# snuspl/parallax

Hardware: NVIDIA H100
Metric: lm1b_words_per_sec (higher is better)
Workload: dtype bf16

## Files before the change

parallax_b200/ops/fused.py:

```python
import ctypes

import torch

from . import lib as _lib, check as _check, register_signatures

_vp, _i, _f = ctypes.c_void_p, ctypes.c_int, ctypes.c_float
register_signatures({
    "px_lstm_cell_fwd": (_i, [_vp, _vp, _vp, _vp, _vp, _i, _i, _f, _i, _vp]),
    "px_lstm_cell_bwd": (_i, [_vp, _vp, _vp, _vp, _vp, _vp, _i, _i, _i, _vp]),
    "px_lstm_dm_cell_bwd": (_i, [_vp] * 7 + [_i, _i, _i, _i, _vp]),
    "px_sampled_softmax": (_i, [_vp, _vp, _vp, _vp, _vp, _vp, _vp, _vp, _i, _i, _i, _vp]),
    "px_sampled_softmax_dot": (_i, [_vp, _vp, _vp, _i, _vp, _vp, _vp, _vp, _vp, _vp, _i, _i, _i,
                                    _vp]),
    "px_ssm_bwd": (_i, [_vp, _vp, _vp, _vp, _i, _vp, _vp, _f, _vp, _vp, _vp, _i, _vp, _i, _i, _i,
                        _vp]),
})
_DT = {torch.float32: 0, torch.bfloat16: 1}


def _p(t):
    return _vp(t.data_ptr())


def _stream():
    return _vp(torch.cuda.current_stream().cuda_stream)


def _count(n=1):
    from ..parallel import nvops
    nvops.launches["n"] += n


def _acc(t):
    return t if t.dtype == torch.float64 else t.float()


BWD_BN = 16


def _fused_bwd_ok(dt, Bsz, S, P, W_P):
    return (dt == torch.bfloat16 and Bsz % 128 == 0 and S % BWD_BN == 0 and P % 64 == 0 and
            W_P.is_contiguous() and W_P.data_ptr() % 16 == 0)


def lstm_layer_reference(x, Wx, Wh, bias, W_P, c0, h0, forget_bias=1.0):
    T, Bsz, E = x.shape
    S = W_P.shape[0]
    xw = torch.addmm(bias, x.reshape(T * Bsz, E), Wx).view(T, Bsz, 4 * S)
    c, h, outs = _acc(c0), h0, []
    for t in range(T):
        gates = _acc(torch.addmm(xw[t], h, Wh))
        i, j, f, o = gates.split(S, dim=1)
        c = torch.sigmoid(f + forget_bias) * c + torch.sigmoid(i) * torch.tanh(j)
        m = (torch.sigmoid(o) * torch.tanh(c)).to(x.dtype)
        h = m @ W_P
        outs.append(h)
    return torch.stack(outs), c, h


class _LSTMLayerFn(torch.autograd.Function):

    @staticmethod
    def forward(ctx, x, W, Wh, bias, W_P, c0, h0, forget_bias):
        L = _lib()
        T, Bsz, E = x.shape
        S, P = W_P.shape
        dt = x.dtype
        dev = x.device
        x = x.contiguous()
        stacked = Wh is None
        ctx.stacked = stacked
        ctx.param_refs = (W, bias, W_P)
        if stacked:
            Wx, Wh = W.detach()[:E], W.detach()[E:]
        else:
            Wx = W
        if any(ctx.needs_input_grad) and not _fused_bwd_ok(dt, Bsz, S, P, W_P):
            from . import sinks
            cur = torch.cuda.current_stream(dev)
            ws = sinks.side_stream(dev)
            ws.wait_stream(cur)
            with torch.cuda.stream(ws):
                ctx.WPT = W_P.detach().t().contiguous()
                ctx.WPT_ev = torch.cuda.Event()
                ctx.WPT_ev.record(ws)
            ctx.WPT.record_stream(cur)
        xw = torch.addmm(bias, x.view(T * Bsz, E), Wx).view(T, Bsz, 4 * S)
        act = torch.empty(T, Bsz, 4 * S, dtype=dt, device=dev)
        c_all = torch.empty(T + 1, Bsz, S, dtype=torch.float32, device=dev)
        m_all = torch.empty(T, Bsz, S, dtype=dt, device=dev)
        h_all = torch.empty(T + 1, Bsz, P, dtype=dt, device=dev)
        c_all[0].copy_(c0)
        h_all[0].copy_(h0)
        st = _stream()
        for t in range(T):
            gpre = xw[t].addmm_(h_all[t], Wh)
            _check(L.px_lstm_cell_fwd(_p(gpre), _p(c_all[t]), _p(act[t]),
                                      _p(c_all[t + 1]), _p(m_all[t]), Bsz, S,
                                      float(forget_bias), _DT[dt], st), "lstm_cell_fwd")
            torch.mm(m_all[t], W_P, out=h_all[t + 1])
        _count(T)
        ctx.save_for_backward(x, Wx, Wh, W_P, act, c_all, m_all, h_all)
        ctx.dims = (T, Bsz, E, S, P)
        return h_all[1:], c_all[T].clone(), h_all[T].clone()

    @staticmethod
    def backward(ctx, dH, dcT, dhT):
        from . import sinks
        L = _lib()
        x, Wx, Wh, W_P, act, c_all, m_all, h_all = ctx.saved_tensors
        T, Bsz, E, S, P = ctx.dims
        stacked = ctx.stacked
        W_ref, bias_ref, WP_ref = ctx.param_refs
        dt, dev = x.dtype, x.device
        dH = dH.contiguous()
        dgates = torch.empty(T, Bsz, 4 * S, dtype=dt, device=dev)
        dh_tot = torch.empty(T, Bsz, P, dtype=dt, device=dev)
        dc = torch.zeros(Bsz, S, dtype=torch.float32, device=dev) if dcT is None \
            else dcT.float().clone()
        dh_rec = None if dhT is None else dhT.to(dt)
        fused = _fused_bwd_ok(dt, Bsz, S, P, W_P)
        dm = None if fused else torch.empty(Bsz, S, dtype=dt, device=dev)
        cur = torch.cuda.current_stream(dev)
        if not fused:
            cur.wait_event(ctx.WPT_ev)
            WPT = ctx.WPT
        from . import gemm as _gemm
        use_tc = (dt == torch.bfloat16 and Bsz % 128 == 0 and P % 64 == 0 and
                  (4 * S) % 1024 == 0 and Wh.is_contiguous())
        WhT = None if use_tc else Wh.t().contiguous()
        st = _stream()

        def sink_of(ref, shape):
            s_ = sinks.get(ref)
            if s_ is not None and s_.dtype == dt and tuple(s_.shape) == tuple(shape):
                return s_, True
            return torch.empty(shape, dtype=dt, device=dev), False
        if stacked:
            dW, w_sunk = sink_of(W_ref, (E + P, 4 * S))
            dWx_o, dWh_o = dW[:E], dW[E:]
        else:
            dWx_o, w_sunk = sink_of(W_ref, (E, 4 * S))
            dWh_o = torch.empty(P, 4 * S, dtype=dt, device=dev)
        dbias_o, b_sunk = sink_of(bias_ref, (4 * S,))
        dWP_o, p_sunk = sink_of(WP_ref, (S, P))
        ws = sinks.side_stream(dev)
        ws2 = sinks.side_stream(dev, 1)
        if dh_rec is None:
            dh_tot[T - 1].copy_(dH[T - 1])
        else:
            torch.add(dH[T - 1], dh_rec, out=dh_tot[T - 1])
        for t in range(T - 1, -1, -1):
            if fused:
                _check(L.px_lstm_dm_cell_bwd(_p(dh_tot[t]), _p(W_P), _p(dc), _p(act[t]),
                                             _p(c_all[t]), _p(c_all[t + 1]), _p(dgates[t]), Bsz,
                                             S, P, BWD_BN, st), "lstm_dm_cell_bwd")
            else:
                torch.mm(dh_tot[t], WPT, out=dm)
                _check(L.px_lstm_cell_bwd(_p(dm), _p(dc), _p(act[t]), _p(c_all[t]),
                                          _p(c_all[t + 1]), _p(dgates[t]), Bsz, S, _DT[dt], st),
                       "lstm_cell_bwd")
            if t > 0:
                if use_tc:
                    _gemm.gemm_tn(dgates[t], Wh, addend=dH[t - 1], splits=8, bn=64,
                                  out=dh_tot[t - 1])
                else:
                    torch.addmm(dH[t - 1], dgates[t], WhT, out=dh_tot[t - 1])
            else:
                dh_rec = _gemm.gemm_tn(dgates[0], Wh, splits=8, bn=64) if use_tc \
                    else torch.mm(dgates[0], WhT)
        _count(T)
        dg2 = dgates.view(T * Bsz, 4 * S)
        ws2.wait_stream(cur)
        with torch.cuda.stream(ws2):
            torch.sum(dg2, 0, out=dbias_o)
        ev_b = torch.cuda.Event()
        ev_b.record(ws2)
        dgates.record_stream(ws2)
        dbias_o.record_stream(ws2)
        dx = (dg2 @ Wx.t()).view(T, Bsz, E)
        ws.wait_stream(cur)
        with torch.cuda.stream(ws):
            torch.mm(h_all[:T].reshape(-1, P).t(), dg2, out=dWh_o)
            torch.mm(x.reshape(-1, E).t(), dg2, out=dWx_o)
            torch.mm(m_all.reshape(-1, S).t(), dh_tot.view(-1, P), out=dWP_o)
        ev = torch.cuda.Event()
        ev.record(ws)
        for t_ in (dgates, dh_tot, x, h_all, m_all, dWh_o, dWx_o, dbias_o, dWP_o):
            t_.record_stream(ws)
        outs, plain = [], False
        for ref, o, sunk, e_ in ((W_ref, dW if stacked else dWx_o, w_sunk, ev),
                                 (bias_ref, dbias_o, b_sunk, ev_b), (WP_ref, dWP_o, p_sunk, ev)):
            if sunk:
                sinks.deliver(ref, e_)
                outs.append(None)
            else:
                outs.append(o)
                plain = True
        if plain or not stacked:
            cur.wait_event(ev)
            cur.wait_event(ev_b)
        dW_out, dbias, dW_P = outs
        return dx, dW_out, None if stacked else dWh_o, dbias, dW_P, dc, dh_rec, None


def lstm_layer(x, Wx, Wh, bias, W_P, c0, h0, forget_bias=1.0):
    if x.is_cuda and x.dtype in _DT:
        return _LSTMLayerFn.apply(x, Wx, Wh, bias, W_P, c0, h0, forget_bias)
    return lstm_layer_reference(x, Wx, Wh, bias, W_P, c0, h0, forget_bias)


def lstm_layer_stacked(x, W, bias, W_P, c0, h0, forget_bias=1.0):
    E = x.shape[-1]
    if x.is_cuda and x.dtype in _DT:
        return _LSTMLayerFn.apply(x, W, None, bias, W_P, c0, h0, forget_bias)
    return lstm_layer_reference(x, W[:E], W[E:], bias, W_P, c0, h0, forget_bias)


def sampled_softmax_reference(inputs, true_w, samp_w, true_b, samp_b, logq_true,
                              logq_samp, targets, sampled):
    true_logits = _acc((inputs * true_w).sum(-1)) + _acc(true_b) - logq_true
    samp_logits = _acc(inputs @ samp_w.t()) + (_acc(samp_b) - logq_samp)
    hits = targets.unsqueeze(1) == sampled.unsqueeze(0)
    samp_logits = samp_logits.masked_fill(hits, float("-inf"))
    lse = torch.logsumexp(torch.cat([true_logits.unsqueeze(1), samp_logits], 1), 1)
    return lse - true_logits


class _SampledSoftmaxFn(torch.autograd.Function):
    @staticmethod
    def forward(ctx, inputs, true_w, samp_w, true_b, samp_b, logq_true, logq_samp,
                targets, sampled):
        L = _lib()
        N, S = inputs.shape[0], samp_w.shape[0]
        dt = inputs.dtype
        logits = inputs @ samp_w.t()
        true_dot = (inputs.float() * true_w.float()).sum(-1)
        adj_t = (true_b.float() - logq_true).contiguous()
        adj_s = (samp_b.float() - logq_samp).contiguous()
        loss = torch.empty(N, dtype=torch.float32, device=inputs.device)
        dtrue = torch.empty(N, dtype=torch.float32, device=inputs.device)
        tg = targets.to(torch.int64).contiguous()
        sm = sampled.to(torch.int64).contiguous()
        _check(L.px_sampled_softmax(_p(logits), _p(true_dot), _p(adj_t), _p(adj_s), _p(tg),
                                    _p(sm), _p(loss), _p(dtrue), N, S, _DT[dt], _stream()),
               "sampled_softmax")
        _count(1)
        ctx.save_for_backward(inputs, true_w, samp_w, logits, dtrue)
        return loss

    @staticmethod
    def backward(ctx, g):
        inputs, true_w, samp_w, probs, dtrue = ctx.saved_tensors
        dt = inputs.dtype
        g = g.float()
        gt = (g * dtrue).unsqueeze(1)
        d_inputs = ((probs @ samp_w).float() * g.unsqueeze(1) +
                    gt * true_w.float()).to(dt)
        gi = (inputs.float() * g.unsqueeze(1)).to(dt)
        d_samp_w = probs.t() @ gi
        d_true_w = (gt * inputs.float()).to(dt)
        d_samp_b = (probs.float().t() @ g) if probs.dtype == torch.float32 else \
            torch.mm(probs.t(), g.to(dt).unsqueeze(1), out_dtype=torch.float32).squeeze(1)
        d_true_b = gt.squeeze(1)
        return d_inputs, d_true_w, d_samp_w, d_true_b, d_samp_b, None, None, None, None


def sampled_softmax_loss(inputs, true_w, samp_w, true_b, samp_b, logq_true, logq_samp,
                         targets, sampled):
    if inputs.is_cuda and inputs.dtype in _DT and samp_w.shape[0] <= 256 * 64:
        return _SampledSoftmaxFn.apply(inputs, true_w.to(inputs.dtype),
                                       samp_w.to(inputs.dtype), true_b, samp_b,
                                       logq_true, logq_samp, targets, sampled)
    return sampled_softmax_reference(inputs, true_w, samp_w, true_b, samp_b, logq_true,
                                     logq_samp, targets, sampled)


def _head_forward(inputs, w_all, adj, targets, sampled):
    N, S = inputs.shape[0], w_all.shape[0] - inputs.shape[0]
    P = inputs.shape[1]
    logits = inputs @ w_all[N:].t()
    if inputs.is_cuda:
        loss = torch.empty(N, dtype=torch.float32, device=inputs.device)
        dtrue = torch.empty(N, dtype=torch.float32, device=inputs.device)
        _check(_lib().px_sampled_softmax_dot(
            _p(logits), _p(inputs), _p(w_all), P, _p(adj), _vp(adj.data_ptr() + 4 * N),
            _p(targets), _p(sampled), _p(loss), _p(dtrue), N, S, _DT[inputs.dtype], _stream()),
            "sampled_softmax_dot")
        _count(1)
        return logits, loss, dtrue
    tl = (inputs.float() * w_all[:N].float()).sum(-1) + adj[:N]
    a = logits.float() + adj[N:]
    a = a.masked_fill(targets.unsqueeze(1) == sampled.unsqueeze(0), float("-inf"))
    mx = torch.maximum(a.max(1).values, tl)
    e, et = torch.exp(a - mx.unsqueeze(1)), torch.exp(tl - mx)
    denom = e.sum(1) + et
    return (e / denom.unsqueeze(1)).to(inputs.dtype), mx + torch.log(denom) - tl, et / denom - 1.0


def _head_backward(G, inputs, w_all, g, row_w, dtrue, gi, d_w_all, db, grow):
    N, P = inputs.shape
    if inputs.is_cuda:
        _check(_lib().px_ssm_bwd(
            _p(G), _p(inputs), _p(w_all), _p(g), 0 if g.numel() == 1 else 1,
            _p(row_w) if row_w is not None else None, _p(dtrue), 1.0 / N, _p(gi), _p(d_w_all),
            _p(db), 1 if db.dtype == torch.bfloat16 else 0, _p(grow), N, P, _DT[inputs.dtype],
            _stream()), "ssm_bwd")
        _count(1)
        return
    gr = g.reshape(-1).float() * (1.0 / N)
    gr = gr.expand(N) if gr.numel() == 1 else gr
    if row_w is not None:
        gr = gr * row_w
    gt = gr * dtrue
    x, wt = inputs.float(), w_all[:N].float()
    G.copy_(G.float() * gr.unsqueeze(1) + gt.unsqueeze(1) * wt)
    gi.copy_(x * gr.unsqueeze(1))
    d_w_all[:N].copy_(x * gt.unsqueeze(1))
    db[:N].copy_(gt)
    grow.copy_(gr)


class _SampledSoftmaxHeadFn(torch.autograd.Function):

    @staticmethod
    def forward(ctx, inputs, w_all, b_all, adj, targets, sampled, row_w):
        probs, loss, dtrue = _head_forward(inputs, w_all, adj, targets, sampled)
        ctx.save_for_backward(inputs, w_all, probs, dtrue, row_w)
        ctx.b_meta = (tuple(b_all.shape), b_all.dtype)
        if row_w is not None:
            loss = loss * row_w
        return loss.mean()

    @staticmethod
    def backward(ctx, g):
        inputs, w_all, probs, dtrue, row_w = ctx.saved_tensors
        N, P = inputs.shape
        S = w_all.shape[0] - N
        dt, dev = inputs.dtype, inputs.device
        b_shape, b_dt = ctx.b_meta
        g = g.float().contiguous()
        G = probs @ w_all[N:]
        d_w_all = torch.empty(N + S, P, dtype=dt, device=dev)
        db = torch.empty(N + S, dtype=b_dt if b_dt in _DT else torch.float32, device=dev)
        gi = torch.empty(N, P, dtype=dt, device=dev)
        grow = torch.empty(N, dtype=dt, device=dev)
        _head_backward(G, inputs, w_all, g, row_w, dtrue, gi, d_w_all, db, grow)
        torch.mm(probs.t(), gi, out=d_w_all[N:])
        if db.dtype == dt:
            torch.mm(probs.t(), grow.view(N, 1), out=db[N:].view(S, 1))
        elif dt == torch.bfloat16 and db.dtype == torch.float32:
            db[N:].copy_(torch.mm(probs.t(), grow.view(N, 1), out_dtype=torch.float32).view(S))
        else:
            db[N:].copy_((probs.t() @ grow.view(N, 1)).view(S))
        db = db.view(b_shape)
        if db.dtype != b_dt:
            db = db.to(b_dt)
        return G, d_w_all, db, None, None, None, None


def sampled_softmax_head(inputs, w_all, b_all, logq, targets, sampled, row_w=None, adj=None):
    N, P = inputs.shape
    S = w_all.shape[0] - N
    dt = inputs.dtype
    vec = 4 if dt == torch.float32 else 8
    fused = (inputs.is_cuda and dt in _DT and w_all.dtype == dt and
             0 < S <= 256 * 64 and P % vec == 0 and b_all.numel() == N + S)
    if fused:
        inputs = inputs.contiguous()
        w_all = w_all.contiguous()
        fused = inputs.data_ptr() % 16 == 0 and w_all.data_ptr() % 16 == 0
    if not fused:
        b = b_all.reshape(-1)
        loss = sampled_softmax_loss(inputs, w_all[:N], w_all[N:], b[:N], b[N:], logq[:N],
                                    logq[N:], targets, sampled)
        if row_w is not None:
            loss = loss * row_w.to(loss.dtype)
        return loss.mean()
    if adj is None:
        adj = b_all.detach().reshape(-1).float() - logq
    adj = adj.float().contiguous()
    tg = targets.to(torch.int64).contiguous()
    sm = sampled.to(torch.int64).contiguous()
    rw = None if row_w is None else row_w.detach().float().contiguous()
    return _SampledSoftmaxHeadFn.apply(inputs, w_all, b_all, adj, tg, sm, rw)
```

Measured before the change: 1.945 million.

## Add persistent cooperative LSTM forward kernel covering all timesteps

Replaces the per-timestep loop of addmm, cell kernel and projection matmul with one cooperative persistent kernel. It keeps recurrent and projection weight slices resident in shared memory, computes gates with wgmma and TMA loads, and uses grid-wide syncs between the gate, projection and split-K reduction phases. The aim is to remove the launch overhead and the repeated weight reloads of 3T launches per layer. In exchange it adds three grid.syncs per step and a split-K fp32 workspace reduction, and it only applies when batch equals BM and the shape constraints fit the grid on the device.

```diff
diff --git a/parallax_b200/ops/csrc/kernels/lstm_persistent.cu b/parallax_b200/ops/csrc/kernels/lstm_persistent.cu
--- /dev/null
+++ b/parallax_b200/ops/csrc/kernels/lstm_persistent.cu
@@ -0,0 +1,305 @@
+#include <cooperative_groups.h>
+#include <mutex>
+
+#include "wgmma.cuh"
+#include "lstm_cell.cuh"
+
+namespace cg = cooperative_groups;
+
+namespace lstm_fwd {
+using namespace tc;
+
+constexpr int UNITS = 32;
+constexpr int ROWS = 64;
+constexpr int GN = 2 * UNITS;
+constexpr int PN = 64;
+constexpr int PK = 128;
+constexpr int NTHREADS = 512;
+constexpr int CELL_U = 4;
+constexpr int GATE_LD = 4 * UNITS + 8;
+constexpr int MAX_KB = 8;
+
+struct Args {
+  const __nv_bfloat16* xw;
+  const __nv_bfloat16* Wh;
+  const __nv_bfloat16* WP;
+  __nv_bfloat16* act;
+  float* c_all;
+  __nv_bfloat16* m_all;
+  __nv_bfloat16* h_all;
+  float* ws;
+  int T, S, P;
+  float forget_bias;
+};
+
+__host__ __device__ constexpr int cmax(int a, int b) { return a > b ? a : b; }
+__host__ __device__ constexpr int x_bytes(int P) {
+  return cmax(cmax((P / BK) * ROWS * 128, (PK / BK) * BM * 128), ROWS * GATE_LD * 4);
+}
+__host__ __device__ constexpr int smem_bytes(int P) {
+  return 2 * (P / BK) * GN * 128 + (PK / BK) * PN * 128 + x_bytes(P) + (MAX_KB + PK / BK) * 8 + 1024;
+}
+static_assert(smem_bytes(MAX_KB * BK) <= 232448, "P = 512 must fit one CTA's shared memory");
+
+template <int N, typename Col>
+__device__ __forceinline__ void load_transposed(uint8_t* dst, const __nv_bfloat16* src, size_t ld,
+                                                int K, Col col) {
+  const int nblk = (N / 8) * (K / 8);
+  for (int b = threadIdx.x; b < nblk; b += blockDim.x) {
+    const int n0 = (b % (N / 8)) * 8, k0 = (b / (N / 8)) * 8;
+    uint4 v[8];
+#pragma unroll
+    for (int i = 0; i < 8; ++i)
+      v[i] = __ldg(reinterpret_cast<const uint4*>(src + (size_t)(k0 + i) * ld + col(n0)));
+    const uint32_t* w = reinterpret_cast<const uint32_t*>(v);
+    uint8_t* blk = dst + (k0 / BK) * N * 128;
+    const int c = (k0 % BK) / 8;
+#pragma unroll
+    for (int j = 0; j < 8; ++j) {
+      const uint32_t sel = (j & 1) ? 0x7632u : 0x5410u;
+      uint4 o;
+      o.x = __byte_perm(w[0 * 4 + j / 2], w[1 * 4 + j / 2], sel);
+      o.y = __byte_perm(w[2 * 4 + j / 2], w[3 * 4 + j / 2], sel);
+      o.z = __byte_perm(w[4 * 4 + j / 2], w[5 * 4 + j / 2], sel);
+      o.w = __byte_perm(w[6 * 4 + j / 2], w[7 * 4 + j / 2], sel);
+      const int n = n0 + j;
+      *reinterpret_cast<uint4*>(blk + n * 128 + ((c ^ (n & 7)) << 4)) = o;
+    }
+  }
+}
+
+__device__ __forceinline__ float2 bf16x2_to_float2(uint32_t w) {
+  return make_float2(__uint_as_float(w << 16), __uint_as_float(w & 0xffff0000u));
+}
+__device__ __forceinline__ uint32_t float2_to_bf16x2(float a, float b) {
+  __nv_bfloat162 h = __floats2bfloat162_rn(a, b);
+  return *reinterpret_cast<uint32_t*>(&h);
+}
+__device__ __forceinline__ float round_bf16(float x) {
+  return __bfloat162float(__float2bfloat16_rn(x));
+}
+
+__device__ __forceinline__ void product(float* acc, uint32_t a0, uint32_t a_stride, uint32_t b0,
+                                        uint64_t* bar, int nkb, uint32_t parity) {
+  for (int kb = 0; kb < nkb; ++kb) {
+    mbar_wait(&bar[kb], parity);
+    const uint64_t adesc = make_smem_desc(a0 + kb * a_stride);
+    const uint64_t bdesc = make_smem_desc(b0 + kb * 64 * 128);
+    wgmma_fence();
+#pragma unroll
+    for (int k = 0; k < BK / WG_K; ++k)
+      wgmma_bf16<64>(acc, adesc + (uint64_t)(k * 2), bdesc + (uint64_t)(k * 2),
+                     (kb | k) != 0 ? 1u : 0u);
+    wgmma_commit();
+  }
+  wgmma_wait<0>();
+}
+
+__global__ void __launch_bounds__(NTHREADS, 1)
+px_lstm_fwd_persistent_kernel(const __grid_constant__ CUtensorMap tmap_h,
+                              const __grid_constant__ CUtensorMap tmap_m, Args a) {
+  extern __shared__ __align__(1024) uint8_t smem_raw[];
+  uint8_t* smem = reinterpret_cast<uint8_t*>(((uintptr_t)smem_raw + 1023) & ~(uintptr_t)1023);
+  const int S = a.S, P = a.P, KB = P / BK;
+  const size_t G4 = 4 * (size_t)S;
+  uint8_t* sWh = smem;
+  uint8_t* sWP = sWh + 2 * KB * GN * 128;
+  uint8_t* sX = sWP + (PK / BK) * PN * 128;
+  uint64_t* hbar = reinterpret_cast<uint64_t*>(sX + x_bytes(P));
+  uint64_t* mbar = hbar + MAX_KB;
+
+  const int row0 = (blockIdx.x & 1) * ROWS, u0 = (blockIdx.x >> 1) * UNITS;
+  const int ntn = P / PN;
+  const bool proj = (int)blockIdx.x < ntn * (S / PK);
+  const int pn0 = (blockIdx.x % ntn) * PN, pk = blockIdx.x / ntn;
+
+  if (threadIdx.x == 0) {
+    asm volatile("prefetch.tensormap [%0];" ::"l"(&tmap_h) : "memory");
+    asm volatile("prefetch.tensormap [%0];" ::"l"(&tmap_m) : "memory");
+    for (int kb = 0; kb < KB; ++kb) mbar_init(&hbar[kb], 1);
+    for (int kb = 0; kb < PK / BK; ++kb) mbar_init(&mbar[kb], 1);
+    asm volatile("fence.mbarrier_init.release.cluster;" ::: "memory");
+  }
+  for (int w = 0; w < 2; ++w)
+    load_transposed<GN>(sWh + w * KB * GN * 128, a.Wh, G4, P,
+                        [=](int n) { return (n / 16) * S + u0 + 16 * w + n % 16; });
+  if (proj)
+    load_transposed<PN>(sWP, a.WP + (size_t)pk * PK * P, P, PK, [=](int n) { return pn0 + n; });
+  asm volatile("fence.proxy.async.shared::cta;" ::: "memory");
+  __syncthreads();
+
+  const int wg = threadIdx.x >> 7, lane = threadIdx.x & 31, warp = (threadIdx.x >> 5) & 3;
+  const int q2 = (lane & 3) * 2;
+  const int r = warp * 16 + (lane >> 2);
+  const int rb = wg * 64 + r;
+  const int crow = threadIdx.x / (UNITS / CELL_U), cu = (threadIdx.x % (UNITS / CELL_U)) * CELL_U;
+  const size_t cs_off = (size_t)(row0 + crow) * S + u0 + cu;
+  const size_t cg_off = (size_t)(row0 + crow) * G4 + u0 + cu;
+  float c[CELL_U];
+  {
+    const float4 v = *reinterpret_cast<const float4*>(a.c_all + cs_off);
+    c[0] = v.x; c[1] = v.y; c[2] = v.z; c[3] = v.w;
+  }
+  float* sG = reinterpret_cast<float*>(sX);
+  const uint32_t sX_u = smem_u32(sX), sWh_u = smem_u32(sWh) + (wg & 1) * KB * GN * 128;
+  const uint32_t sWP_u = smem_u32(sWP);
+  cg::grid_group grid = cg::this_grid();
+  const int KS = S / PK;
+  float acc[32];
+
+  for (int t = 0; t < a.T; ++t) {
+    const uint32_t parity = t & 1;
+    if (threadIdx.x == 0) {
+      asm volatile("fence.proxy.async.global;" ::: "memory");
+      for (int kb = 0; kb < KB; ++kb) {
+        mbar_expect_tx(&hbar[kb], ROWS * BK * 2);
+        tma_load_2d(sX + kb * ROWS * 128, &tmap_h, &hbar[kb], kb * BK, t * BM + row0);
+      }
+    }
+    uint2 xv[4];
+    const __nv_bfloat16* xr = a.xw + (size_t)t * BM * G4 + cg_off;
+#pragma unroll
+    for (int g = 0; g < 4; ++g) xv[g] = __ldg(reinterpret_cast<const uint2*>(xr + (size_t)g * S));
+    if (wg < 2) {
+      product(acc, sX_u, ROWS * 128, sWh_u, hbar, KB, parity);
+      consumer_sync();
+#pragma unroll
+      for (int h = 0; h < 2; ++h)
+#pragma unroll
+        for (int j = 0; j < GN / 8; ++j)
+          *reinterpret_cast<float2*>(sG + (r + 8 * h) * GATE_LD + (j >> 1) * UNITS + wg * 16 +
+                                     (j & 1) * 8 + q2) =
+              make_float2(acc[j * 4 + 2 * h], acc[j * 4 + 2 * h + 1]);
+    }
+    __syncthreads();
+
+    float av[4][CELL_U], mv[CELL_U];
+#pragma unroll
+    for (int g = 0; g < 4; ++g) {
+      const float4 v = *reinterpret_cast<const float4*>(sG + crow * GATE_LD + g * UNITS + cu);
+      const float2 lo = bf16x2_to_float2(xv[g].x), hi = bf16x2_to_float2(xv[g].y);
+      av[g][0] = round_bf16(v.x + lo.x);
+      av[g][1] = round_bf16(v.y + lo.y);
+      av[g][2] = round_bf16(v.z + hi.x);
+      av[g][3] = round_bf16(v.w + hi.y);
+    }
+    asm volatile("fence.proxy.async.shared::cta;" ::: "memory");
+#pragma unroll
+    for (int e = 0; e < CELL_U; ++e) {
+      float ae[4];
+      c[e] = lstm_cell_fwd_elem(av[0][e], av[1][e], av[2][e], av[3][e], c[e], a.forget_bias, ae,
+                                &mv[e]);
+#pragma unroll
+      for (int g = 0; g < 4; ++g) av[g][e] = ae[g];
+    }
+    __nv_bfloat16* act = a.act + (size_t)t * BM * G4 + cg_off;
+#pragma unroll
+    for (int g = 0; g < 4; ++g)
+      *reinterpret_cast<uint2*>(act + (size_t)g * S) =
+          make_uint2(float2_to_bf16x2(av[g][0], av[g][1]), float2_to_bf16x2(av[g][2], av[g][3]));
+    *reinterpret_cast<float4*>(a.c_all + (size_t)(t + 1) * BM * S + cs_off) =
+        make_float4(c[0], c[1], c[2], c[3]);
+    *reinterpret_cast<uint2*>(a.m_all + (size_t)t * BM * S + cs_off) =
+        make_uint2(float2_to_bf16x2(mv[0], mv[1]), float2_to_bf16x2(mv[2], mv[3]));
+    grid.sync();
+
+    if (proj && wg < 2) {
+      if (threadIdx.x == 0) {
+        asm volatile("fence.proxy.async.global;" ::: "memory");
+        for (int kb = 0; kb < PK / BK; ++kb) {
+          mbar_expect_tx(&mbar[kb], BM * BK * 2);
+          tma_load_2d(sX + kb * BM * 128, &tmap_m, &mbar[kb], pk * PK + kb * BK, t * BM);
+        }
+      }
+      product(acc, sX_u + wg * 64 * 128, BM * 128, sWP_u, mbar, PK / BK, parity);
+      float* slot = a.ws + (size_t)pk * BM * P;
+#pragma unroll
+      for (int h = 0; h < 2; ++h)
+#pragma unroll
+        for (int j = 0; j < PN / 8; ++j)
+          *reinterpret_cast<float2*>(slot + (size_t)(rb + 8 * h) * P + pn0 + j * 8 + q2) =
+              make_float2(acc[j * 4 + 2 * h], acc[j * 4 + 2 * h + 1]);
+    }
+    grid.sync();
+
+    __nv_bfloat16* hn = a.h_all + (size_t)(t + 1) * BM * P;
+    const int npairs = BM * P / 2;
+    for (int i = blockIdx.x * blockDim.x + threadIdx.x; i < npairs; i += gridDim.x * blockDim.x) {
+      float2 s = __ldcg(reinterpret_cast<const float2*>(a.ws) + i);
+#pragma unroll 8
+      for (int k = 1; k < KS; ++k) {
+        const float2 v = __ldcg(reinterpret_cast<const float2*>(a.ws + (size_t)k * BM * P) + i);
+        s.x += v.x;
+        s.y += v.y;
+      }
+      reinterpret_cast<uint32_t*>(hn)[i] = float2_to_bf16x2(s.x, s.y);
+    }
+    if (t + 1 < a.T) grid.sync();
+  }
+}
+
+}
+
+extern "C" {
+
+int px_lstm_fwd_persistent_grid(int B, int S, int P) {
+  using namespace lstm_fwd;
+  if (B != BM || S <= 0 || S % PK || P <= 0 || P % PN || P > MAX_KB * BK) return 0;
+  static std::mutex mu;
+  static int cap[16][MAX_KB + 1];
+  int dev = 0;
+  if (cudaGetDevice(&dev) != cudaSuccess || dev < 0 || dev >= 16) return 0;
+  std::lock_guard<std::mutex> lock(mu);
+  int& n = cap[dev][P / PN];
+  if (n == 0) {
+    int coop = 0, sms = 0, per_sm = 0;
+    cudaDeviceGetAttribute(&coop, cudaDevAttrCooperativeLaunch, dev);
+    cudaDeviceGetAttribute(&sms, cudaDevAttrMultiProcessorCount, dev);
+    const int smem = smem_bytes(P);
+    if (cudaFuncSetAttribute(px_lstm_fwd_persistent_kernel,
+                             cudaFuncAttributeMaxDynamicSharedMemorySize,
+                             smem_bytes(MAX_KB * BK)) != cudaSuccess ||
+        cudaOccupancyMaxActiveBlocksPerMultiprocessor(&per_sm, px_lstm_fwd_persistent_kernel,
+                                                      NTHREADS, smem) != cudaSuccess)
+      per_sm = 0;
+    n = (coop && per_sm > 0) ? per_sm * sms : -1;
+    cudaGetLastError();
+  }
+  const int grid = 2 * (S / UNITS);
+  return n >= grid ? grid : 0;
+}
+
+int px_lstm_fwd_persistent(const void* xw, const void* Wh, const void* WP, void* act, float* c_all,
+                           void* m_all, void* h_all, float* ws, int T, int B, int S, int P,
+                           float forget_bias, cudaStream_t stream) {
+  using namespace lstm_fwd;
+  const int grid = px_lstm_fwd_persistent_grid(B, S, P);
+  if (grid <= 0 || T < 1) return -1;
+  for (const void* q : {xw, Wh, WP, (const void*)act, (const void*)c_all, (const void*)m_all,
+                        (const void*)h_all, (const void*)ws})
+    if ((uintptr_t)q % 16) return -1;
+  CUtensorMap th, tm;
+  int rc = make_tmap(&th, h_all, (uint64_t)(T + 1) * B, P, ROWS);
+  if (rc) return rc;
+  rc = make_tmap(&tm, m_all, (uint64_t)T * B, S, BM);
+  if (rc) return rc;
+  Args a;
+  a.xw = (const __nv_bfloat16*)xw; a.Wh = (const __nv_bfloat16*)Wh;
+  a.WP = (const __nv_bfloat16*)WP; a.act = (__nv_bfloat16*)act; a.c_all = c_all;
+  a.m_all = (__nv_bfloat16*)m_all; a.h_all = (__nv_bfloat16*)h_all; a.ws = ws;
+  a.T = T; a.S = S; a.P = P; a.forget_bias = forget_bias;
+  cudaLaunchConfig_t cfg = {};
+  cfg.gridDim = dim3(grid);
+  cfg.blockDim = dim3(NTHREADS);
+  cfg.dynamicSmemBytes = smem_bytes(P);
+  cfg.stream = stream;
+  cudaLaunchAttribute at[1];
+  at[0].id = cudaLaunchAttributeCooperative;
+  at[0].val.cooperative = 1;
+  cfg.attrs = at;
+  cfg.numAttrs = 1;
+  const cudaError_t e = cudaLaunchKernelEx(&cfg, px_lstm_fwd_persistent_kernel, th, tm, a);
+  return e == cudaSuccess ? (int)cudaGetLastError() : (int)e;
+}
+
+}
diff --git a/parallax_b200/ops/fused.py b/parallax_b200/ops/fused.py
--- a/parallax_b200/ops/fused.py
+++ b/parallax_b200/ops/fused.py
@@ -9,6 +9,8 @@
     "px_lstm_cell_fwd": (_i, [_vp, _vp, _vp, _vp, _vp, _i, _i, _f, _i, _vp]),
     "px_lstm_cell_bwd": (_i, [_vp, _vp, _vp, _vp, _vp, _vp, _i, _i, _i, _vp]),
     "px_lstm_dm_cell_bwd": (_i, [_vp] * 7 + [_i, _i, _i, _i, _vp]),
+    "px_lstm_fwd_persistent_grid": (_i, [_i, _i, _i]),
+    "px_lstm_fwd_persistent": (_i, [_vp] * 8 + [_i, _i, _i, _i, _f, _vp]),
     "px_sampled_softmax": (_i, [_vp, _vp, _vp, _vp, _vp, _vp, _vp, _vp, _i, _i, _i, _vp]),
     "px_sampled_softmax_dot": (_i, [_vp, _vp, _vp, _i, _vp, _vp, _vp, _vp, _vp, _vp, _i, _i, _i,
                                     _vp]),
@@ -41,6 +43,19 @@
 def _fused_bwd_ok(dt, Bsz, S, P, W_P):
     return (dt == torch.bfloat16 and Bsz % 128 == 0 and S % BWD_BN == 0 and P % 64 == 0 and
             W_P.is_contiguous() and W_P.data_ptr() % 16 == 0)
+
+
+_persistent_grid = {}
+
+
+def _fwd_persistent_ok(dt, Bsz, S, P, Wh, W_P):
+    if not (dt == torch.bfloat16 and Wh.is_contiguous() and W_P.is_contiguous() and
+            Wh.data_ptr() % 16 == 0 and W_P.data_ptr() % 16 == 0):
+        return False
+    key = (torch.cuda.current_device(), Bsz, S, P)
+    if key not in _persistent_grid:
+        _persistent_grid[key] = _lib().px_lstm_fwd_persistent_grid(Bsz, S, P)
+    return _persistent_grid[key] > 0
 
 
 def lstm_layer_reference(x, Wx, Wh, bias, W_P, c0, h0, forget_bias=1.0):
@@ -93,13 +108,20 @@
         c_all[0].copy_(c0)
         h_all[0].copy_(h0)
         st = _stream()
-        for t in range(T):
-            gpre = xw[t].addmm_(h_all[t], Wh)
-            _check(L.px_lstm_cell_fwd(_p(gpre), _p(c_all[t]), _p(act[t]),
-                                      _p(c_all[t + 1]), _p(m_all[t]), Bsz, S,
-                                      float(forget_bias), _DT[dt], st), "lstm_cell_fwd")
-            torch.mm(m_all[t], W_P, out=h_all[t + 1])
-        _count(T)
+        if _fwd_persistent_ok(dt, Bsz, S, P, Wh, W_P):
+            ws = torch.empty(S // 128, Bsz, P, dtype=torch.float32, device=dev)
+            _check(L.px_lstm_fwd_persistent(_p(xw), _p(Wh), _p(W_P), _p(act), _p(c_all),
+                                            _p(m_all), _p(h_all), _p(ws), T, Bsz, S, P,
+                                            float(forget_bias), st), "lstm_fwd_persistent")
+            _count(1)
+        else:
+            for t in range(T):
+                gpre = xw[t].addmm_(h_all[t], Wh)
+                _check(L.px_lstm_cell_fwd(_p(gpre), _p(c_all[t]), _p(act[t]),
+                                          _p(c_all[t + 1]), _p(m_all[t]), Bsz, S,
+                                          float(forget_bias), _DT[dt], st), "lstm_cell_fwd")
+                torch.mm(m_all[t], W_P, out=h_all[t + 1])
+            _count(T)
         ctx.save_for_backward(x, Wx, Wh, W_P, act, c_all, m_all, h_all)
         ctx.dims = (T, Bsz, E, S, P)
         return h_all[1:], c_all[T].clone(), h_all[T].clone()
```

Result: faster. 2.011 million, median of 6 (+3.4%).
